# laboshinl/loam_velodyne

Measured on AMD Instinct MI355X. Metric: sweeps/sec (64-ring, 1M-pt map): feature extraction + odometry + scan-to-map registration, higher is better.
Workload: dtype f32

## Files before the change

loam_velodyne_amd/csrc/features.hip:

```cpp
#include "features.hpp"
#include "pinned_copy.hpp"
#include "scan.hpp"

namespace loamx {

__device__ inline float sqdiff3(const float4& a, const float4& b) {
  const float dx = a.x - b.x, dy = a.y - b.y, dz = a.z - b.z;
  return dx * dx + dy * dy + dz * dz;
}
__device__ inline float sqdiff3w(const float4& a, const float4& b, float wb) {
  const float dx = a.x - b.x * wb, dy = a.y - b.y * wb, dz = a.z - b.z * wb;
  return dx * dx + dy * dy + dz * dz;
}

struct RingLds {
  uint8_t* flags;
  float* c;
  uint32_t* sorted;
  int8_t* label;
};

__device__ inline void wave_lds_sync() { __builtin_amdgcn_fence(__ATOMIC_ACQ_REL, "workgroup"); }

__device__ inline void mark_as_picked(uint32_t scan_i, int cr, uint8_t* flags, const uint8_t* gaps, int lane) {
// ... 271 lines not shown
        if (!(ep > sp) || ep - sp + 1 < (unsigned long long)cr) simple = 0;
      }
      s_simple = simple && !force_sequential;
    }
    float* c = (float*)(wave_base + wid * wave_bytes);
    uint32_t* sorted = (uint32_t*)(c + nmax);
    int8_t* label = (int8_t*)(sorted + nmax);
    for (int jb = 0; jb < nreg; jb += FEAT_WAVES) {
      const int j = jb + wid;
      uint32_t n = 0, gsp = 0, scan_sp = 0;
      if (j < nreg) {
        const unsigned long long sp = ((s0 + cr) * (unsigned long long)(nreg - j) + (e0 - cr) * (unsigned long long)j) / nreg;
        const unsigned long long ep = ((s0 + cr) * (unsigned long long)(nreg - 1 - j) + (e0 - cr) * (unsigned long long)(j + 1)) / nreg - 1;
        if (ep > sp) {
          n = (uint32_t)(ep - sp + 1);
          gsp = base + (uint32_t)sp;
          scan_sp = (uint32_t)(sp - s0);
        }
      }
      if (lane == 0) { reg_n[wid] = n; reg_gsp[wid] = gsp; reg_scan[wid] = scan_sp; }
      for (uint32_t e = lane; e < n; e += 64) {
        c[e] = curv_all[scan_sp + e];
        label[e] = 0;
      }
      if (lane < 4 && n) c[n + lane] = __builtin_inff();
      __syncthreads();
      FT_TS(1);
      if (sortP == 64) wave_sort_curvature<1>(c, n, sorted, lane);
      else if (sortP == 128) wave_sort_curvature<2>(c, n, sorted, lane);
      else if (sortP == 256) wave_sort_curvature<4>(c, n, sorted, lane);
      else if (sortP == 512) wave_sort_curvature<8>(c, n, sorted, lane);
      else if (wid < (int)nwaves) {
        unsigned long long* keys = (unsigned long long*)(wave_base + nwaves * wave_bytes + (size_t)wid * sortP * 8);
        for (uint32_t e = lane; e < sortP; e += 64)
          keys[e] = e < n ? ((unsigned long long)__float_as_uint(c[e]) << 32) | e : ~0ull;
        wave_lds_sync();
        for (uint32_t k = 2; k <= sortP; k <<= 1) {
          for (uint32_t j = k >> 1; j > 0; j >>= 1) {
            for (uint32_t t = lane; t < sortP / 2; t += 64) {
              const uint32_t i = ((t / j) * 2 * j) + (t % j), l = i + j;
              const unsigned long long a = keys[i], b = keys[l];
              const bool up = (i & k) == 0;
              if ((a > b) == up) { keys[i] = b; keys[l] = a; }
            }
            wave_lds_sync();
          }
        }
        for (uint32_t e = lane; e < n; e += 64) sorted[e] = (uint32_t)keys[e];
      }
      __syncthreads();
      FT_TS(2);
      if (s_simple) {
        const uint32_t rn = reg_n[wid];
        if (rn) {
          if (wid == 0 && jb > 0)
            for (uint32_t e = lane; e < (uint32_t)cr && e < rn; e += 64) flags[reg_scan[0] + e] |= fwd[reg_scan[0] + e];
          wave_lds_sync();
          region_picks(P, cr, rn, reg_gsp[wid], reg_scan[wid], c, sorted, label, flags, fwd, gaps, pickS + (size_t)j * P.max_sharp,
                       pickLS + (size_t)j * P.max_less_sharp, pickF + (size_t)j * P.max_flat, rcnt[j], lane);
        }
        __syncthreads();
        if (wid == 0) {
          for (int w = 1; w < FEAT_WAVES && jb + w < nreg; w++) {
            const uint32_t rn2 = reg_n[w], rscan2 = reg_scan[w], rgsp2 = reg_gsp[w];
            const float* rc = (const float*)(wave_base + w * wave_bytes);
            const uint32_t* rsorted = (const uint32_t*)(rc + nmax);
            int8_t* rlabel = (int8_t*)(rsorted + nmax);
            const bool hit = lane < cr && (uint32_t)lane < rn2 && fwd[rscan2 + lane] != 0 && rlabel[lane] != 0;
            if (__ballot(hit)) {
              for (uint32_t e = lane; e < rn2; e += 64) {
                flags[rscan2 + e] = flags0[rscan2 + e] | (e < (uint32_t)cr ? fwd[rscan2 + e] : (uint8_t)0);
                rlabel[e] = 0;
              }
              for (uint32_t e = lane; e < (uint32_t)cr; e += 64) fwd[rscan2 + rn2 + e] = 0;
              wave_lds_sync();
              region_picks(P, cr, rn2, rgsp2, rscan2, rc, rsorted, rlabel, flags, fwd, gaps, pickS + (size_t)(jb + w) * P.max_sharp,
                           pickLS + (size_t)(jb + w) * P.max_less_sharp, pickF + (size_t)(jb + w) * P.max_flat, rcnt[jb + w], lane);
            }
          }
        }
      } else if (wid == 0) {
        for (int w = 0; w < FEAT_WAVES && jb + w < nreg; w++) {
          const uint32_t rn2 = reg_n[w];
          if (rn2 == 0) continue;
          const float* rc = (const float*)(wave_base + w * wave_bytes);
          const uint32_t* rsorted = (const uint32_t*)(rc + nmax);
          int8_t* rlabel = (int8_t*)(rsorted + nmax);
          region_picks(P, cr, rn2, reg_gsp[w], reg_scan[w], rc, rsorted, rlabel, flags, nullptr, gaps, pickS + (size_t)(jb + w) * P.max_sharp,
                       pickLS + (size_t)(jb + w) * P.max_less_sharp, pickF + (size_t)(jb + w) * P.max_flat, rcnt[jb + w], lane);
        }
      }
      __syncthreads();
      FT_TS(3);
      for (uint32_t e = lane; e < n; e += 64) lf_valid[gsp + e] = label[e] <= 0 ? 1 : 0;
      __syncthreads();
    }
  }
  if (wid == 0 && len > 2u * cr + 1u) {
    uint32_t* lists[3] = {pickS, pickLS, pickF};
    const uint32_t per[3] = {(uint32_t)P.max_sharp, (uint32_t)P.max_less_sharp, (uint32_t)P.max_flat};
    uint32_t tot[3] = {0, 0, 0};
    for (int j = 0; j < nreg; j++) {
#pragma unroll
      for (int q = 0; q < 3; q++) {
        const uint32_t cnt = rcnt[j][q], src = (uint32_t)j * per[q];
        if (src != tot[q]) {
          for (uint32_t k0 = 0; k0 < cnt; k0 += 64) {
            const uint32_t k = k0 + lane;
            const uint32_t v = k < cnt ? lists[q][src + k] : 0u;
            wave_lds_sync();
            if (k < cnt) lists[q][tot[q] + k] = v;
            wave_lds_sync();
          }
        }
        tot[q] += cnt;
      }
    }
    nS = tot[0]; nLS = tot[1]; nF = tot[2];
  }
  if (tid == 0) {
    cntS[r] = nS;
    cntLS[r] = nLS;
    cntF[r] = nF;
    npick[0] = nS; npick[1] = nLS; npick[2] = nF;
  }
  __syncthreads();
  for (uint32_t k = tid; k < npick[0]; k += blockDim.x) slotS[(size_t)r * capS + k] = cloud[pickS[k]];
  for (uint32_t k = tid; k < npick[1]; k += blockDim.x) slotLS[(size_t)r * capLS + k] = cloud[pickLS[k]];
  for (uint32_t k = tid; k < npick[2]; k += blockDim.x) slotF[(size_t)r * capF + k] = cloud[pickF[k]];
  FT_TS(4);
}

struct FeatRingLds {
  uint32_t flag_bytes, nmax, sortP, nwaves;
  size_t bytes;
};
constexpr size_t FEAT_LDS_STATIC = 1024;
constexpr size_t FEAT_LDS_MAX = 160 * 1024 - FEAT_LDS_STATIC;
static_assert(sizeof(uint32_t) * (3 * FEAT_WAVES + 3 + 64 * 3) + sizeof(int) <= FEAT_LDS_STATIC, "k_feat_ring's static LDS");

static FeatRingLds feat_ring_lds(uint32_t max_len, const FeatParams& p) {
  FeatRingLds r;
  const size_t caps = (size_t)(p.max_sharp + p.max_less_sharp + p.max_flat) * p.n_regions;
  r.flag_bytes = (max_len + 15u) & ~15u;
  r.nmax = (max_len / (uint32_t)p.n_regions + 8u + 15u) & ~15u;
  r.sortP = 64;
  while (r.sortP < r.nmax) r.sortP <<= 1;
  r.nwaves = (uint32_t)std::min(p.n_regions, FEAT_WAVES);
  r.bytes = ((8 * (size_t)r.flag_bytes + 4 * caps + 15) & ~(size_t)15) + (size_t)r.nwaves * r.nmax * (4 + 4 + 1) +
            (r.sortP > 512 ? (size_t)r.nwaves * r.sortP * 8 : 0) + 16;
  return r;
}

constexpr int LFV_THREADS = 1024;
constexpr uint32_t LFV_MAX = 4096;

__global__ __launch_bounds__(LFV_THREADS) void k_feat_lf_voxel(const float4* __restrict__ cloud, const uint32_t* __restrict__ ring_off,
                                                               const uint8_t* __restrict__ lf_valid, float inv_leaf, uint32_t P,
                                                               float4* __restrict__ slots, uint32_t* __restrict__ cnt) {
  extern __shared__ __attribute__((aligned(16))) char smem[];
  unsigned long long* keys = (unsigned long long*)smem;
  __shared__ uint32_t sc[17];
  __shared__ int mm[6];
  __shared__ uint32_t s_wcnt[LFV_THREADS / 64][256];
  __shared__ uint32_t s_base[256];
  const uint32_t r = blockIdx.x, tid = threadIdx.x;
  const uint32_t s0 = ring_off[r], len = ring_off[r + 1] - s0;
  if (tid < 3) mm[tid] = 2147483647;
  else if (tid < 6) mm[tid] = -2147483647 - 1;
  for (uint32_t k = tid; k < P; k += LFV_THREADS) keys[k] = ~0ull;
  __syncthreads();
  uint32_t base = 0;
  for (uint32_t b = 0; b < len; b += LFV_THREADS) {
    const uint32_t i = b + tid;
    const uint32_t v = (i < len && lf_valid[s0 + i]) ? 1u : 0u;
    uint32_t total;
    const uint32_t ex = block_excl_scan(v, sc, total);
    if (v) keys[base + ex] = i;
    base += total;
  }
  const uint32_t m = base;
  __syncthreads();
  {
    int lo[3] = {2147483647, 2147483647, 2147483647}, hi[3] = {-2147483647 - 1, -2147483647 - 1, -2147483647 - 1};
    for (uint32_t j = tid; j < m; j += LFV_THREADS) {
      const float4 p = cloud[s0 + (uint32_t)keys[j]];
      const int c[3] = {(int)floorf(p.x * inv_leaf), (int)floorf(p.y * inv_leaf), (int)floorf(p.z * inv_leaf)};
#pragma unroll
      for (int a = 0; a < 3; a++) { lo[a] = min(lo[a], c[a]); hi[a] = max(hi[a], c[a]); }
    }
#pragma unroll
    for (int off = 32; off > 0; off >>= 1) {
#pragma unroll
      for (int a = 0; a < 3; a++) {
        lo[a] = min(lo[a], __shfl_xor(lo[a], off, 64));
        hi[a] = max(hi[a], __shfl_xor(hi[a], off, 64));
      }
    }
    if ((tid & 63u) == 0) {
#pragma unroll
      for (int a = 0; a < 3; a++) { atomicMin(&mm[a], lo[a]); atomicMax(&mm[3 + a], hi[a]); }
    }
  }
  __syncthreads();
  const long long dx = (long long)mm[3] - mm[0] + 1, dy = (long long)mm[4] - mm[1] + 1, dz = (long long)mm[5] - mm[2] + 1;
  const bool pass = m > 0 && (dx > 2147483647LL || dy > 2147483647LL || dx * dy > 2147483647LL || dz > 2147483647LL / (dx * dy) + 1 || dx * dy * dz > 2147483647LL);
  for (uint32_t j = tid; j < m; j += LFV_THREADS) {
    const uint32_t li = (uint32_t)keys[j];
    unsigned long long k;
    if (pass) {
      k = (unsigned long long)j;
    } else {
      const float4 p = cloud[s0 + li];
      const int jx = (int)floorf(p.x * inv_leaf), jy = (int)floorf(p.y * inv_leaf), jz = (int)floorf(p.z * inv_leaf);
      k = (unsigned long long)((long long)(jx - mm[0]) + (long long)(jy - mm[1]) * dx + (long long)(jz - mm[2]) * dx * dy);
    }
    keys[j] = (k << 12) | li;
  }
  __syncthreads();
  unsigned long long* kb[2] = {keys, (unsigned long long*)(smem + (size_t)P * 8)};
  uint32_t npass = 0;
  if (!pass && m > 1) {
    const unsigned long long top = (unsigned long long)(dx * dy * dz - 1);
    const uint32_t bits = top ? 64u - (uint32_t)__builtin_clzll(top) : 0u;
    npass = (bits + 7u) / 8u;
  }
  {
    const uint32_t lane = tid & 63u, wid = tid >> 6;
    const uint32_t per_wave = ((m + LFV_THREADS - 1) / LFV_THREADS) * 64u;
    for (uint32_t ps = 0; ps < npass; ps++) {
      const uint32_t shift = 12u + 8u * ps;
      const unsigned long long* src = kb[ps & 1];
      unsigned long long* dst = kb[(ps & 1) ^ 1];
      for (uint32_t e = tid; e < (LFV_THREADS / 64) * 256; e += LFV_THREADS) (&s_wcnt[0][0])[e] = 0u;
      __syncthreads();
      unsigned long long key[4];
      uint32_t rank[4];
#pragma unroll
      for (int j = 0; j < 4; j++) {
        const uint32_t i = wid * per_wave + (uint32_t)j * 64u + lane;
        const bool in = (uint32_t)j * 64u < per_wave && i < m;
        key[j] = in ? src[i] : ~0ull;
        const uint32_t d = (uint32_t)((key[j] >> shift) & 255ull);
        unsigned long long mt = __ballot(in);
#pragma unroll
        for (int b = 0; b < 8; b++) {
          const unsigned long long bal = __ballot((d >> b) & 1u);
          mt &= ((d >> b) & 1u) ? bal : ~bal;
        }
        const unsigned long long below = mt & ((1ull << lane) - 1ull);
        const int leader = __builtin_ctzll(mt | (1ull << 63));
        uint32_t old = 0u;
        if (in && (int)lane == leader) {
          old = s_wcnt[wid][d];
          s_wcnt[wid][d] = old + (uint32_t)__popcll(mt);
        }
        old = __shfl(old, leader, 64);
        rank[j] = old + (uint32_t)__popcll(below);
        __builtin_amdgcn_wave_barrier();
      }
      __syncthreads();
      uint32_t run = 0;
      if (tid < 256) {
#pragma unroll
        for (int w = 0; w < LFV_THREADS / 64; w++) { const uint32_t c = s_wcnt[w][tid]; s_wcnt[w][tid] = run; run += c; }
      }
      uint32_t tot;
      const uint32_t ex = block_excl_scan(run, sc, tot);
      if (tid < 256) s_base[tid] = ex;
      __syncthreads();
#pragma unroll
      for (int j = 0; j < 4; j++) {
        const uint32_t i = wid * per_wave + (uint32_t)j * 64u + lane;
        if ((uint32_t)j * 64u < per_wave && i < m) {
          const uint32_t d = (uint32_t)((key[j] >> shift) & 255ull);
          dst[s_base[d] + s_wcnt[wid][d] + rank[j]] = key[j];
        }
      }
      __syncthreads();
    }
    if (npass & 1u) {
      for (uint32_t j = tid; j < m; j += LFV_THREADS) keys[j] = kb[1][j];
      __syncthreads();
    }
  }
  float4* sp = (float4*)(smem + (size_t)P * 8);
  for (uint32_t j = tid; j < m; j += LFV_THREADS) sp[j] = cloud[s0 + (uint32_t)(keys[j] & 4095ull)];
  __syncthreads();
  uint32_t obase = 0;
  for (uint32_t b = 0; b < m; b += LFV_THREADS) {
    const uint32_t j = b + tid;
    const bool head = j < m && (j == 0 || (keys[j] >> 12) != (keys[j - 1] >> 12));
    uint32_t total;
    const uint32_t ex = block_excl_scan(head ? 1u : 0u, sc, total);
    if (head) {
      const unsigned long long vk = keys[j] >> 12;
      float sx = 0.f, sy = 0.f, sz = 0.f, si = 0.f;
      uint32_t e = j;
      do {
        const float4 p = sp[e];
        sx += p.x; sy += p.y; sz += p.z; si += p.w;
        e++;
      } while (e < m && (keys[e] >> 12) == vk);
      const float c = (float)(e - j);
      slots[s0 + obase + ex] = make_float4(sx / c, sy / c, sz / c, si / c);
    }
    obase += total;
  }
  if (tid == 0) cnt[r] = obase;
}

__device__ inline uint32_t rings_before(const uint32_t* __restrict__ c, uint32_t r, int lane) {
  uint32_t part = 0u;
  for (uint32_t i = (uint32_t)lane; i < r; i += 64u) part += c[i];
#pragma unroll
  for (int d = 32; d > 0; d >>= 1) part += (uint32_t)__shfl_xor((int)part, d, 64);
  return part;
}
__global__ __launch_bounds__(64) void k_feat_compact(const float4* __restrict__ s0, const float4* __restrict__ s1, const float4* __restrict__ s2,
                                                     const uint32_t* __restrict__ c0, const uint32_t* __restrict__ c1, const uint32_t* __restrict__ c2,
                                                     uint32_t cap0, uint32_t cap1, uint32_t cap2, float4* __restrict__ o0, float4* __restrict__ o1,
                                                     float4* __restrict__ o2, uint32_t* __restrict__ offs, const uint32_t* __restrict__ sweep_ring_base,
                                                     uint32_t nsw, uint32_t* __restrict__ host_offs) {
  const uint32_t r = blockIdx.x, kind = blockIdx.y, nring = gridDim.x;
  const int lane = (int)threadIdx.x;
  const float4* s = kind == 0 ? s0 : (kind == 1 ? s1 : s2);
  const uint32_t* c = kind == 0 ? c0 : (kind == 1 ? c1 : c2);
  const uint32_t cap = kind == 0 ? cap0 : (kind == 1 ? cap1 : cap2);
  float4* o = kind == 0 ? o0 : (kind == 1 ? o1 : o2);
  const uint32_t dst = rings_before(c, r, lane), n = c[r];
  for (uint32_t k = (uint32_t)lane; k < n; k += 64u) o[dst + k] = s[(size_t)r * cap + k];
  if (lane == 0) {
    uint32_t* off = offs + (size_t)kind * (nsw + 1);
    uint32_t* hoff = host_offs ? host_offs + (size_t)kind * (nsw + 1) : nullptr;
    uint32_t lo = 0, hi = nsw + 1;
    while (lo < hi) { const uint32_t mid = (lo + hi) >> 1; if (sweep_ring_base[mid] < r) lo = mid + 1; else hi = mid; }
    for (uint32_t sw = lo; sw <= nsw && sweep_ring_base[sw] == r; sw++) { off[sw] = dst; if (hoff) hoff[sw] = dst; }
    if (r + 1 == nring)
      for (uint32_t sw = nsw; sweep_ring_base[sw] >= nring; sw--) { off[sw] = dst + n; if (hoff) hoff[sw] = dst + n; if (sw == 0) break; }
  }
}
__global__ __launch_bounds__(256) void k_feat_lf_compact(const float4* __restrict__ slots, const uint32_t* __restrict__ ring_off,
                                                         const uint32_t* __restrict__ cnt, uint32_t* __restrict__ lf_off, float4* __restrict__ out,
                                                         uint32_t* __restrict__ host_lf_off) {
  __shared__ uint32_t s_dst;
  const uint32_t r = blockIdx.x;
  if (threadIdx.x < 64) {
    const uint32_t d = rings_before(cnt, r, (int)threadIdx.x);
    if (threadIdx.x == 0) {
      s_dst = d;
      lf_off[r] = d;
      if (r + 1 == gridDim.x) lf_off[gridDim.x] = d + cnt[r];
      if (host_lf_off) {
        host_lf_off[r] = d;
        if (r + 1 == gridDim.x) host_lf_off[gridDim.x] = d + cnt[r];
      }
    }
  }
  __syncthreads();
  const uint32_t n = cnt[r], src = ring_off[r], dst = s_dst;
  for (uint32_t k = threadIdx.x; k < n; k += blockDim.x) out[dst + k] = slots[src + k];
}

FeatureExtractor::FeatureExtractor(int device, hipStream_t shared_stream) : device_(device) {
  select_device(device);
  if (shared_stream) {
    st_ = shared_stream;
  } else {
    LX_HIP(hipStreamCreateWithFlags(&st_, hipStreamNonBlocking));
    own_stream_ = true;
  }
  vox_.init(st_);
  h_bad_.reserve(16);
  h_bad_.p[0] = 0u;
  h_bad_.p[1] = 0u;
}

void FeatureExtractor::check_finite_input() {
  if (*(volatile uint32_t*)h_bad_.p) {
    *h_bad_.p = 0u;
    throw Error(LOAMX_E_INVALID, "a sweep holds non-finite coordinates (binned rings must be finite: BasicLaserOdometry.cpp:230 / MultiScanRegistration.cpp:187-196 drop such points before this stage)");
  }
}

FeatureExtractor::~FeatureExtractor() {
  if (ev_front_) (void)hipEventDestroy(ev_front_);
  if (ev_lf_) (void)hipEventDestroy(ev_lf_);
  if (own_stream_ && st_) (void)hipStreamDestroy(st_);
}

void FeatureExtractor::check_params_() const {
  LX_REQUIRE(params.curv_region >= 1 && params.curv_region <= 16, "curvature_region must be in [1,16]");
  LX_REQUIRE(params.n_regions >= 1 && params.n_regions <= 64, "n_feature_regions must be in [1,64]");
  LX_REQUIRE(params.max_sharp >= 0 && params.max_flat >= 0 && params.max_less_sharp >= params.max_sharp, "invalid pick limits");
  LX_REQUIRE(params.less_flat_leaf > 0.f, "less_flat_filter_size must be positive");
}

void FeatureExtractor::upload_async(uint32_t nsw, const loamx_cloud* clouds, const uint32_t* const* ring_size, const uint32_t* n_rings,
                                    hipStream_t copy_stream, hipEvent_t done, const std::function<bool(void*, const void*, size_t)>& big_copy) {
  LX_REQUIRE(nsw >= 1 && clouds && ring_size && n_rings && copy_stream && done, "invalid sweep batch");
  check_params_();
  LX_HIP(hipSetDevice(device_));
  bool packed = true;
  for (uint32_t s = 0; s < nsw; s++) {
    check_cloud(&clouds[s], false);
    uint32_t sum = 0;
    for (uint32_t r = 0; r < n_rings[s]; r++) sum += ring_size[s][r];
    LX_REQUIRE(sum == clouds[s].count, "ring sizes do not add up to the cloud size");
    packed = packed && clouds[s].stride == 16 && clouds[s].intensity_offset == 12;
  }
  layout_(nsw, ring_size, n_rings);
  allocate_(copy_stream);
  if (packed) {
    for (uint32_t s = 0; s < nsw;) {
      uint32_t e = s + 1;
      size_t cnt = clouds[s].count;
      while (e < nsw && (const char*)clouds[e].data == (const char*)clouds[s].data + sizeof(float4) * cnt) cnt += clouds[e++].count;
      if (cnt && !(big_copy && big_copy(cloud_.p + h_pt_base_[s], clouds[s].data, sizeof(float4) * cnt)))
        LX_HIP(hipMemcpyAsync(cloud_.p + h_pt_base_[s], clouds[s].data, sizeof(float4) * cnt, hipMemcpyHostToDevice, copy_stream));
      s = e;
    }
  } else {
    h_cloud_.reserve(n_ + 1);
    for (uint32_t s = 0; s < nsw; s++) pack_cloud(&clouds[s], h_cloud_.p + h_pt_base_[s]);
    if (n_) LX_HIP(hipMemcpyAsync(cloud_.p, h_cloud_.p, sizeof(float4) * n_, hipMemcpyHostToDevice, copy_stream));
  }
  LX_HIP(hipEventRecord(done, copy_stream));
}
void FeatureExtractor::upload_device(uint32_t nsw, const float4* d_src, const uint32_t* src_off, const uint32_t* const* ring_size,
                                     const uint32_t* n_rings, hipStream_t copy_stream, hipEvent_t done) {
  LX_REQUIRE(nsw >= 1 && d_src && src_off && ring_size && n_rings && copy_stream && done, "invalid sweep batch");
  check_params_();
  LX_HIP(hipSetDevice(device_));
  layout_(nsw, ring_size, n_rings);
  allocate_(copy_stream);
  for (uint32_t s = 0; s < nsw; s++) {
    const uint32_t cnt = h_pt_base_[s + 1] - h_pt_base_[s];
    if (cnt) LX_HIP(hipMemcpyAsync(cloud_.p + h_pt_base_[s], d_src + src_off[s], sizeof(float4) * cnt, hipMemcpyDeviceToDevice, copy_stream));
  }
  LX_HIP(hipEventRecord(done, copy_stream));
}
void FeatureExtractor::layout_(uint32_t nsw, const uint32_t* const* ring_size, const uint32_t* n_rings) {
  uint32_t longest = 0;
  for (uint32_t s = 0; s < nsw; s++)
    for (uint32_t r = 0; r < n_rings[s]; r++) longest = std::max(longest, ring_size[s][r]);
  LX_REQUIRE(feat_ring_lds(longest, params).bytes <= FEAT_LDS_MAX, "scan ring too long for the LDS staging of k_feat_ring (include/loamx.h)");
  nsw_ = nsw;
  h_ring_off_.assign(1, 0);
  h_ring_base_.assign(nsw + 1, 0);
  h_pt_base_.assign(nsw + 1, 0);
  h_ring_sweep_base_.clear();
  max_ring_len_ = 0;
  uint32_t pt = 0;
  for (uint32_t s = 0; s < nsw; s++) {
    uint32_t sum = 0;
    for (uint32_t r = 0; r < n_rings[s]; r++) {
      sum += ring_size[s][r];
      h_ring_off_.push_back(pt + sum);
      h_ring_sweep_base_.push_back(pt);
      max_ring_len_ = std::max(max_ring_len_, ring_size[s][r]);
    }
    pt += sum;
// ... 120 lines not shown
    imu_.fill_table(h_imu_d_.p, h_imu_f_.p, I);
    imu_dt_.reserve(2 * (size_t)H);
    imu_state_.reserve(9 * (size_t)H);
    imu_last_.reserve(1);
    h_imu_last_.reserve(1);
    LX_HIP(hipMemcpyAsync(imu_dt_.p, h_imu_d_.p, sizeof(double) * 2 * H, hipMemcpyHostToDevice, st_));
    LX_HIP(hipMemcpyAsync(imu_state_.p, h_imu_f_.p, sizeof(float) * 9 * H, hipMemcpyHostToDevice, st_));
    LX_HIP(hipMemsetAsync(imu_last_.p, 0, sizeof(ImuLast), st_));
    I.dt = imu_dt_.p;
    I.dstamp = imu_dt_.p + H;
    I.state = imu_state_.p;
  }
  return H;
}

void FeatureExtractor::finish_raw_(uint32_t n_scan_rings, uint32_t H) {
  LX_HIP(hipMemcpyAsync(h_raw_ring_cnt_.p, raw_ring_cnt_.p, sizeof(uint32_t) * n_scan_rings, hipMemcpyDeviceToHost, st_));
  if (H) LX_HIP(hipMemcpyAsync(h_imu_last_.p, imu_last_.p, sizeof(ImuLast), hipMemcpyDeviceToHost, st_));
  LX_HIP(hipStreamSynchronize(st_));
  if (H && h_imu_last_.p->valid) imu_.apply_last(*h_imu_last_.p);
  begin_sweep();
  const uint32_t* rs[1] = {h_raw_ring_cnt_.p};
  layout_(1, rs, &n_scan_rings);
  allocate_();
  LX_HIP(hipStreamSynchronize(st_));
}

void ImuTracker::update(double stamp, float roll, float pitch, float yaw, const float acc_in[3]) {
  State st;
  st.stamp = stamp; st.roll = HAngle(roll); st.pitch = HAngle(pitch); st.yaw = HAngle(yaw);
  st.acceleration = {acc_in[0], acc_in[1], acc_in[2]};
  if (!hist_.empty()) {
    HVec3 acc = st.acceleration;
    h_rot_zxy(acc, st.roll, st.pitch, st.yaw);
    const State& prev = hist_.back();
    const float dt = (float)(stamp - prev.stamp);
    st.position = {prev.position.x + prev.velocity.x * dt + 0.5f * acc.x * dt * dt, prev.position.y + prev.velocity.y * dt + 0.5f * acc.y * dt * dt,
                   prev.position.z + prev.velocity.z * dt + 0.5f * acc.z * dt * dt};
    st.velocity = {prev.velocity.x + acc.x * dt, prev.velocity.y + acc.y * dt, prev.velocity.z + acc.z * dt};
  }
  if (hist_.size() >= (size_t)std::max(history_size, 1)) hist_.pop_front();
  hist_.push_back(st);
}

void ImuTracker::interpolate_for_(float rel, State& out) {
  double td = (scan_time_ - hist_[idx_].stamp) + rel;
  while (idx_ < hist_.size() - 1 && td > 0) {
    idx_++;
    td = (scan_time_ - hist_[idx_].stamp) + rel;
  }
  if (idx_ == 0 || td > 0) {
    out = hist_[idx_];
  } else {
    const State &a = hist_[idx_], &b = hist_[idx_ - 1];
    const float ratio = (float)(-td / (a.stamp - b.stamp)), inv = 1 - ratio;
    out.roll = HAngle(a.roll.r * inv + b.roll.r * ratio);
    out.pitch = HAngle(a.pitch.r * inv + b.pitch.r * ratio);
    if (a.yaw.r - b.yaw.r > M_PI) out.yaw = HAngle((float)(a.yaw.r * inv + (b.yaw.r + 2 * M_PI) * ratio));
    else if (a.yaw.r - b.yaw.r < -M_PI) out.yaw = HAngle((float)(a.yaw.r * inv + (b.yaw.r - 2 * M_PI) * ratio));
    else out.yaw = HAngle(a.yaw.r * inv + b.yaw.r * ratio);
    out.velocity = {a.velocity.x * inv + b.velocity.x * ratio, a.velocity.y * inv + b.velocity.y * ratio, a.velocity.z * inv + b.velocity.z * ratio};
    out.position = {a.position.x * inv + b.position.x * ratio, a.position.y * inv + b.position.y * ratio, a.position.z * inv + b.position.z * ratio};
  }
}

void ImuTracker::begin_sweep() {
  scan_time_ = next_scan_time_;
  idx_ = 0;
  if (!hist_.empty()) interpolate_for_(0.f, start_);
  sweep_start_ = scan_time_;
  imu_trans_[0] = start_.pitch.r; imu_trans_[1] = start_.yaw.r; imu_trans_[2] = start_.roll.r;
  imu_trans_[3] = cur_.pitch.r; imu_trans_[4] = cur_.yaw.r; imu_trans_[5] = cur_.roll.r;
  HVec3 sh = shift_;
  h_rot_yxz(sh, -start_.yaw, -start_.pitch, -start_.roll);
  imu_trans_[6] = sh.x; imu_trans_[7] = sh.y; imu_trans_[8] = sh.z;
  HVec3 v{cur_.velocity.x - start_.velocity.x, cur_.velocity.y - start_.velocity.y, cur_.velocity.z - start_.velocity.z};
  h_rot_yxz(v, -start_.yaw, -start_.pitch, -start_.roll);
  imu_trans_[9] = v.x; imu_trans_[10] = v.y; imu_trans_[11] = v.z;
}

void ImuTracker::fill_table(double* h_d, float* h_f, ImuTable& I) const {
  const uint32_t H = (uint32_t)hist_.size();
  for (uint32_t j = 0; j < H; j++) {
    const State& s = hist_[j];
    h_d[j] = scan_time_ - s.stamp;
    h_d[H + j] = j ? s.stamp - hist_[j - 1].stamp : 1.0;
    float* o = h_f + 9 * (size_t)j;
    o[0] = s.roll.r; o[1] = s.pitch.r; o[2] = s.yaw.r;
    o[3] = s.position.x; o[4] = s.position.y; o[5] = s.position.z;
    o[6] = s.velocity.x; o[7] = s.velocity.y; o[8] = s.velocity.z;
  }
  I.H = H;
  I.idx0 = H ? (uint32_t)std::min(idx_, (size_t)H - 1) : 0u;
  const HAngle* sa[3] = {&start_.roll, &start_.pitch, &start_.yaw};
  for (int k = 0; k < 3; k++) { I.start_c[k] = sa[k]->c; I.start_s[k] = sa[k]->s; }
  I.start_pos[0] = start_.position.x; I.start_pos[1] = start_.position.y; I.start_pos[2] = start_.position.z;
  I.start_vel[0] = start_.velocity.x; I.start_vel[1] = start_.velocity.y; I.start_vel[2] = start_.velocity.z;
  I.rel_sweep_base = scan_time_ - sweep_start_;
}

void ImuTracker::apply_last(const ImuLast& L) {
  cur_.roll = HAngle(L.roll); cur_.pitch = HAngle(L.pitch); cur_.yaw = HAngle(L.yaw);
  cur_.position = {L.pos[0], L.pos[1], L.pos[2]};
  cur_.velocity = {L.vel[0], L.vel[1], L.vel[2]};
  shift_ = {L.shift[0], L.shift[1], L.shift[2]};
  idx_ = L.idx;
}

int FeatureExtractor::download_cloud(uint32_t sweep, loamx_cloud* full, uint32_t* ring_size_out) {
  LX_REQUIRE(sweep < nsw_, "sweep index out of range");
  const uint32_t r0 = h_ring_base_[sweep], r1 = h_ring_base_[sweep + 1];
  if (ring_size_out)
    for (uint32_t r = r0; r < r1; r++) ring_size_out[r - r0] = h_ring_off_[r + 1] - h_ring_off_[r];
  if (!full) return LOAMX_OK;
  check_cloud(full, false);
  const uint32_t a = h_pt_base_[sweep], b = h_pt_base_[sweep + 1];
  h_pack_.reserve((size_t)(b - a) + 2);
  if (b > a) LX_HIP(hipMemcpyAsync(h_pack_.p, cloud_.p + a, sizeof(float4) * (b - a), hipMemcpyDeviceToHost, st_));
  LX_HIP(hipStreamSynchronize(st_));
  return unpack_cloud(h_pack_.p, b - a, full);
}

void FeatureExtractor::run_async(bool mirror_offsets) {
  TraceRange trace_range("loamx:features:extract");
  LX_REQUIRE(nsw_ > 0, "run() before upload()");
  LX_HIP(hipSetDevice(device_));
  split_ = mirror_offsets && max_ring_len_ <= LFV_MAX;
  uint32_t* hmir = nullptr;
  if (split_) {
    h_mirror_off_.reserve(n_offsets());
    hmir = h_mirror_off_.p;
    if (!ev_front_) { LX_HIP(hipEventCreateWithFlags(&ev_front_, hipEventDisableTiming)); LX_HIP(hipEventCreateWithFlags(&ev_lf_, hipEventDisableTiming)); }
  }
  const int cr = params.curv_region;
  (void)cr;
  const uint32_t caps[3] = {(uint32_t)(params.max_sharp * params.n_regions), (uint32_t)(params.max_less_sharp * params.n_regions),
                            (uint32_t)(params.max_flat * params.n_regions)};
  const FeatRingLds L = feat_ring_lds(max_ring_len_, params);
  const size_t lds = L.bytes;
  LX_REQUIRE(lds <= FEAT_LDS_MAX, "internal: scan ring too long for the LDS staging of k_feat_ring");
  static const bool force_seq = diag_env("LOAMX_FEAT_SEQUENTIAL") && atoi(diag_env("LOAMX_FEAT_SEQUENTIAL")) != 0;
  if (lds > 64 * 1024)
    LX_HIP(hipFuncSetAttribute((const void*)k_feat_ring, hipFuncAttributeMaxDynamicSharedMemorySize, (int)lds));
  hipLaunchKernelGGL(k_feat_ring, dim3(nring_), dim3(64 * FEAT_WAVES), lds, st_, cloud_.p, ring_off_.p, ring_sweep_base_.p, params, L.flag_bytes, L.nmax,
                     L.sortP, L.nwaves, slots_[0].p, slots_[1].p, slots_[2].p, slot_cnt_[0].p, slot_cnt_[1].p, slot_cnt_[2].p, lf_valid_.p, force_seq ? 1 : 0,
                     h_bad_.p);
  hipLaunchKernelGGL(k_feat_compact, dim3(nring_, 3), dim3(64), 0, st_, slots_[0].p, slots_[1].p, slots_[2].p, slot_cnt_[0].p, slot_cnt_[1].p,
                     slot_cnt_[2].p, caps[0], caps[1], caps[2], out_[0].p, out_[1].p, out_[2].p, offs_.p, sweep_ring_base_.p, nsw_, hmir);
  if (split_) LX_HIP(hipEventRecord(ev_front_, st_));
  const float inv = 1.0f / params.less_flat_leaf;
  if (max_ring_len_ <= LFV_MAX) {
    uint32_t P = 2;
    while (P < max_ring_len_) P <<= 1;
    if ((size_t)P * 24 > 64 * 1024)
      LX_HIP(hipFuncSetAttribute((const void*)k_feat_lf_voxel, hipFuncAttributeMaxDynamicSharedMemorySize, (int)((size_t)P * 24)));
    hipLaunchKernelGGL(k_feat_lf_voxel, dim3(nring_), dim3(LFV_THREADS), (size_t)P * 24, st_, cloud_.p, ring_off_.p, lf_valid_.p, inv, P,
                       lf_slots_.p, lf_cnt_.p);
    hipLaunchKernelGGL(k_feat_lf_compact, dim3(nring_), dim3(256), 0, st_, lf_slots_.p, ring_off_.p, lf_cnt_.p, lf_off_(), lf_out_.p,
                       hmir ? hmir + (size_t)3 * off_stride_ : nullptr);
    if (split_) LX_HIP(hipEventRecord(ev_lf_, st_));
  } else {
    vox_.compute_ijk(cloud_.p, lf_valid_.p, n_, ring_off_.p, nring_, inv, inv);
    vox_.sort_reduce(cloud_.p, lf_valid_.p, n_, ring_off_.p, nring_, lf_out_.p, lf_off_());
  }
#ifdef LOAMX_PROF_FEAT
  {
    unsigned long long ts[8];
    LX_HIP(hipStreamSynchronize(st_));
    LX_HIP(hipMemcpyFromSymbol(ts, HIP_SYMBOL(g_feat_ts), sizeof(ts)));
    fprintf(stderr, "[feat_ring ts, 10ns ticks] load %lld  rank-sort %lld  picks %lld  tail %lld\n", (long long)(ts[1] - ts[0]), (long long)(ts[2] - ts[1]),
            (long long)(ts[3] - ts[2]), (long long)(ts[4] - ts[3]));
  }
#endif
  LX_HIP(hipGetLastError());
}

void FeatureExtractor::sync() {
  LX_HIP(hipStreamSynchronize(st_));
  vox_.check();
  check_finite_input();
}

__global__ __launch_bounds__(256) void k_feat_pack_host(const float4* __restrict__ o0, const float4* __restrict__ o1, const float4* __restrict__ o2,
                                                        const float4* __restrict__ lf, const uint32_t* __restrict__ off0,
                                                        const uint32_t* __restrict__ off1, const uint32_t* __restrict__ off2,
                                                        const uint32_t* __restrict__ lf_off, uint32_t sweep, uint32_t ring_a, uint32_t ring_b,
                                                        uint32_t capacity, float4* __restrict__ dst) {
  const uint32_t a0 = off0[sweep], n0 = off0[sweep + 1] - a0, a1 = off1[sweep], n1 = off1[sweep + 1] - a1;
  const uint32_t a2 = off2[sweep], n2 = off2[sweep + 1] - a2, a3 = lf_off[ring_a], n3 = lf_off[ring_b] - a3;
  const uint32_t total = n0 + n1 + n2 + n3;
  if (blockIdx.x == 0 && threadIdx.x == 0) {
    uint4 h = make_uint4(n0, n1, n2, n3);
    if (total > capacity) h = make_uint4(0xffffffffu, 0xffffffffu, 0xffffffffu, 0xffffffffu);
    *reinterpret_cast<uint4*>(dst) = h;
  }
  if (total > capacity) return;
  for (uint32_t i = blockIdx.x * blockDim.x + threadIdx.x; i < total; i += gridDim.x * blockDim.x) {
    float4 v;
    if (i < n0) v = o0[a0 + i];
    else if (i < n0 + n1) v = o1[a1 + (i - n0)];
    else if (i < n0 + n1 + n2) v = o2[a2 + (i - n0 - n1)];
    else v = lf[a3 + (i - n0 - n1 - n2)];
    dst[1 + i] = v;
  }
}

void FeatureExtractor::device_results(uint32_t sweep, const float4* ptr[4], uint32_t count[4]) {
  LX_REQUIRE(sweep < nsw_, "sweep index out of range");
  h_link_off_.reserve(n_offsets());
  LX_HIP(hipMemcpyAsync(h_link_off_.p, offs_.p, sizeof(uint32_t) * n_offsets(), hipMemcpyDeviceToHost, st_));
  LX_HIP(hipStreamSynchronize(st_));
  vox_.check();
  check_finite_input();
  const uint32_t* o = h_link_off_.p;
  for (int k = 0; k < 3; k++) {
    const uint32_t a = o[(size_t)k * off_stride_ + sweep], b = o[(size_t)k * off_stride_ + sweep + 1];
    ptr[k] = out_[k].p + a;
    count[k] = b - a;
  }
  const uint32_t* lf = o + (size_t)3 * off_stride_;
  const uint32_t a = lf[h_ring_base_[sweep]], b = lf[h_ring_base_[sweep + 1]];
  ptr[3] = lf_out_.p + a;
  count[3] = b - a;
}

void FeatureExtractor::device_results_front(uint32_t sweep, const float4* ptr[3], uint32_t count[3]) {
  LX_REQUIRE(sweep < nsw_, "sweep index out of range");
  LX_REQUIRE(split_, "internal: device_results_front() without run_async(true)");
  spin_event(ev_front_);
  check_finite_input();
  const uint32_t* o = h_mirror_off_.p;
  for (int k = 0; k < 3; k++) {
    const uint32_t a = o[(size_t)k * off_stride_ + sweep], b = o[(size_t)k * off_stride_ + sweep + 1];
    ptr[k] = out_[k].p + a;
    count[k] = b - a;
  }
}
void FeatureExtractor::device_results_lf(uint32_t sweep, const float4*& ptr, uint32_t& count) {
  LX_REQUIRE(sweep < nsw_, "sweep index out of range");
  LX_REQUIRE(split_, "internal: device_results_lf() without run_async(true)");
  spin_event(ev_lf_);
  const uint32_t* lf = h_mirror_off_.p + (size_t)3 * off_stride_;
  const uint32_t a = lf[h_ring_base_[sweep]], b = lf[h_ring_base_[sweep + 1]];
  ptr = lf_out_.p + a;
  count = b - a;
}

int FeatureExtractor::download(uint32_t sweep, loamx_cloud* sharp, loamx_cloud* less_sharp, loamx_cloud* flat, loamx_cloud* less_flat) {
  LX_REQUIRE(sweep < nsw_, "sweep index out of range");
  loamx_cloud* outs[4] = {sharp, less_sharp, flat, less_flat};
  for (auto* o : outs) if (o) check_cloud(o, false);
  const uint32_t n_pts = h_pt_base_[sweep + 1] - h_pt_base_[sweep];
  const uint32_t capacity = 4 * n_pts;
  h_pack_.reserve((size_t)capacity + 2);
  hipLaunchKernelGGL(k_feat_pack_host, dim3(std::min<uint32_t>((capacity + 1023) / 1024 + 1, 128u)), dim3(256), 0, st_, out_[0].p, out_[1].p, out_[2].p,
                     lf_out_.p, d_feat_off(0), d_feat_off(1), d_feat_off(2), lf_off_(), sweep, h_ring_base_[sweep], h_ring_base_[sweep + 1], capacity,
                     h_pack_.p);
  LX_HIP(hipStreamSynchronize(st_));
  vox_.check();
  check_finite_input();
  const uint32_t* hdr = reinterpret_cast<const uint32_t*>(h_pack_.p);
  LX_REQUIRE(hdr[0] != 0xffffffffu, "internal: the feature clouds of a sweep exceed four times its points");
  int rc = LOAMX_OK;
  const float4* src = h_pack_.p + 1;
  for (int k = 0; k < 4; k++) {
    if (outs[k]) {
      const int r = unpack_cloud(src, hdr[k], outs[k]);
      if (r != LOAMX_OK) rc = r;
    }
    src += hdr[k];
  }
  return rc;
}

}
```

Baseline: 16840.

## Restructure per-ring less-flat voxel kernel with LDS point staging and fewer block scans

Rewrites the per-ring voxel-downsample kernel to use 256 threads, each owning a contiguous chunk of points. Valid points are compacted with a single block scan and staged into LDS once, so the key and mean phases no longer reload from global memory. Head detection and the output base offsets use one wave-level scan instead of a block scan per chunk. The radix rank step drops the leader shuffle, and the mean accumulation is unrolled by four. It also adds an early exit for empty rings and optional profiling timestamps, at the cost of more LDS per block (32 bytes per slot instead of 24) and fewer threads per ring.

Result: no change. 16830 (-0.0%).

```diff
diff --git a/loam_velodyne_amd/csrc/features.hip b/loam_velodyne_amd/csrc/features.hip
--- a/loam_velodyne_amd/csrc/features.hip
+++ b/loam_velodyne_amd/csrc/features.hip
@@ -447,42 +447,76 @@
   return r;
 }
 
-constexpr int LFV_THREADS = 1024;
+constexpr int LFV_THREADS = 256;
 constexpr uint32_t LFV_MAX = 4096;
+constexpr int LFV_WAVES = LFV_THREADS / 64;
+constexpr int LFV_SLOTS = (int)LFV_MAX / LFV_THREADS;
+constexpr int LFV_LOADS = 8;
+static_assert(LFV_THREADS >= 256 && LFV_THREADS <= 1024 && LFV_WAVES * LFV_SLOTS == 64, "the 256 digits and the 64 head counts are scanned by one thread each");
+
+#ifdef LOAMX_PROF_FEAT
+__device__ unsigned long long g_lfv_ts[8];
+#define LFV_TS(k) do { if (blockIdx.x == 100 && threadIdx.x == 0) g_lfv_ts[k] = wall_clock64(); } while (0)
+#else
+#define LFV_TS(k) do { } while (0)
+#endif
 
 __global__ __launch_bounds__(LFV_THREADS) void k_feat_lf_voxel(const float4* __restrict__ cloud, const uint32_t* __restrict__ ring_off,
                                                                const uint8_t* __restrict__ lf_valid, float inv_leaf, uint32_t P,
                                                                float4* __restrict__ slots, uint32_t* __restrict__ cnt) {
   extern __shared__ __attribute__((aligned(16))) char smem[];
-  unsigned long long* keys = (unsigned long long*)smem;
+  float4* pts = (float4*)smem;
+  unsigned long long* kb0 = (unsigned long long*)(smem + (size_t)P * 16);
+  unsigned long long* kb1 = kb0 + P;
+  uint32_t* idx = (uint32_t*)kb1;
   __shared__ uint32_t sc[17];
   __shared__ int mm[6];
-  __shared__ uint32_t s_wcnt[LFV_THREADS / 64][256];
-  __shared__ uint32_t s_base[256];
-  const uint32_t r = blockIdx.x, tid = threadIdx.x;
+  __shared__ uint32_t s_wcnt[LFV_WAVES][256];
+  __shared__ uint32_t s_heads[64];
+  const uint32_t r = blockIdx.x, tid = threadIdx.x, lane = tid & 63u, wid = tid >> 6;
   const uint32_t s0 = ring_off[r], len = ring_off[r + 1] - s0;
+  LFV_TS(0);
   if (tid < 3) mm[tid] = 2147483647;
   else if (tid < 6) mm[tid] = -2147483647 - 1;
-  for (uint32_t k = tid; k < P; k += LFV_THREADS) keys[k] = ~0ull;
-  __syncthreads();
-  uint32_t base = 0;
-  for (uint32_t b = 0; b < len; b += LFV_THREADS) {
-    const uint32_t i = b + tid;
-    const uint32_t v = (i < len && lf_valid[s0 + i]) ? 1u : 0u;
-    uint32_t total;
-    const uint32_t ex = block_excl_scan(v, sc, total);
-    if (v) keys[base + ex] = i;
-    base += total;
-  }
-  const uint32_t m = base;
+  if (tid < 64) s_heads[tid] = 0u;
+  const uint32_t C = (len + LFV_THREADS - 1) / LFV_THREADS, first = tid * C;
+  uint32_t own = 0u;
+#pragma unroll
+  for (int c = 0; c < LFV_SLOTS; c++) {
+    const uint32_t i = first + (uint32_t)c;
+    if ((uint32_t)c < C && i < len && lf_valid[s0 + i]) own |= 1u << c;
+  }
+  uint32_t m;
+  {
+    uint32_t at = block_excl_scan((uint32_t)__popc(own), sc, m);
+    while (own) {
+      idx[at++] = first + (uint32_t)__builtin_ctz(own);
+      own &= own - 1u;
+    }
+  }
+  if (m == 0u) {
+    if (tid == 0) cnt[r] = 0u;
+    return;
+  }
   __syncthreads();
   {
     int lo[3] = {2147483647, 2147483647, 2147483647}, hi[3] = {-2147483647 - 1, -2147483647 - 1, -2147483647 - 1};
-    for (uint32_t j = tid; j < m; j += LFV_THREADS) {
-      const float4 p = cloud[s0 + (uint32_t)keys[j]];
-      const int c[3] = {(int)floorf(p.x * inv_leaf), (int)floorf(p.y * inv_leaf), (int)floorf(p.z * inv_leaf)};
-#pragma unroll
-      for (int a = 0; a < 3; a++) { lo[a] = min(lo[a], c[a]); hi[a] = max(hi[a], c[a]); }
+    for (uint32_t b = 0; b < m; b += LFV_LOADS * LFV_THREADS) {
+      uint32_t li[LFV_LOADS];
+      float4 p[LFV_LOADS];
+#pragma unroll
+      for (int k = 0; k < LFV_LOADS; k++) li[k] = idx[min(b + (uint32_t)k * LFV_THREADS + tid, m - 1u)];
+#pragma unroll
+      for (int k = 0; k < LFV_LOADS; k++) p[k] = cloud[s0 + li[k]];
+#pragma unroll
+      for (int k = 0; k < LFV_LOADS; k++) {
+        if (b + (uint32_t)k * LFV_THREADS + tid < m) {
+          pts[li[k]] = p[k];
+          const int c[3] = {(int)floorf(p[k].x * inv_leaf), (int)floorf(p[k].y * inv_leaf), (int)floorf(p[k].z * inv_leaf)};
+#pragma unroll
+          for (int a = 0; a < 3; a++) { lo[a] = min(lo[a], c[a]); hi[a] = max(hi[a], c[a]); }
+        }
+      }
     }
 #pragma unroll
     for (int off = 32; off > 0; off >>= 1) {
@@ -492,51 +526,54 @@
         hi[a] = max(hi[a], __shfl_xor(hi[a], off, 64));
       }
     }
-    if ((tid & 63u) == 0) {
+    if (lane == 0) {
 #pragma unroll
       for (int a = 0; a < 3; a++) { atomicMin(&mm[a], lo[a]); atomicMax(&mm[3 + a], hi[a]); }
     }
   }
   __syncthreads();
+  LFV_TS(1);
   const long long dx = (long long)mm[3] - mm[0] + 1, dy = (long long)mm[4] - mm[1] + 1, dz = (long long)mm[5] - mm[2] + 1;
-  const bool pass = m > 0 && (dx > 2147483647LL || dy > 2147483647LL || dx * dy > 2147483647LL || dz > 2147483647LL / (dx * dy) + 1 || dx * dy * dz > 2147483647LL);
+  const bool pass = dx > 2147483647LL || dy > 2147483647LL || dx * dy > 2147483647LL || dz > 2147483647LL / (dx * dy) + 1 || dx * dy * dz > 2147483647LL;
   for (uint32_t j = tid; j < m; j += LFV_THREADS) {
-    const uint32_t li = (uint32_t)keys[j];
+    const uint32_t li = idx[j];
     unsigned long long k;
     if (pass) {
       k = (unsigned long long)j;
     } else {
-      const float4 p = cloud[s0 + li];
+      const float4 p = pts[li];
       const int jx = (int)floorf(p.x * inv_leaf), jy = (int)floorf(p.y * inv_leaf), jz = (int)floorf(p.z * inv_leaf);
       k = (unsigned long long)((long long)(jx - mm[0]) + (long long)(jy - mm[1]) * dx + (long long)(jz - mm[2]) * dx * dy);
     }
-    keys[j] = (k << 12) | li;
+    kb0[j] = (k << 12) | li;
   }
   __syncthreads();
-  unsigned long long* kb[2] = {keys, (unsigned long long*)(smem + (size_t)P * 8)};
+  LFV_TS(2);
+#ifdef LOAMX_PROF_FEAT
+  if (blockIdx.x == 100 && tid == 0) g_lfv_ts[3] = g_lfv_ts[4] = g_lfv_ts[5] = g_lfv_ts[6] = 0ull;
+#endif
   uint32_t npass = 0;
   if (!pass && m > 1) {
     const unsigned long long top = (unsigned long long)(dx * dy * dz - 1);
     const uint32_t bits = top ? 64u - (uint32_t)__builtin_clzll(top) : 0u;
     npass = (bits + 7u) / 8u;
   }
-  {
-    const uint32_t lane = tid & 63u, wid = tid >> 6;
-    const uint32_t per_wave = ((m + LFV_THREADS - 1) / LFV_THREADS) * 64u;
-    for (uint32_t ps = 0; ps < npass; ps++) {
-      const uint32_t shift = 12u + 8u * ps;
-      const unsigned long long* src = kb[ps & 1];
-      unsigned long long* dst = kb[(ps & 1) ^ 1];
-      for (uint32_t e = tid; e < (LFV_THREADS / 64) * 256; e += LFV_THREADS) (&s_wcnt[0][0])[e] = 0u;
-      __syncthreads();
-      unsigned long long key[4];
-      uint32_t rank[4];
-#pragma unroll
-      for (int j = 0; j < 4; j++) {
+  const uint32_t per_wave = ((m + LFV_THREADS - 1) / LFV_THREADS) * 64u;
+  for (uint32_t ps = 0; ps < npass; ps++) {
+    const uint32_t shift = 12u + 8u * ps;
+    const unsigned long long* src = (ps & 1u) ? kb1 : kb0;
+    unsigned long long* dst = (ps & 1u) ? kb0 : kb1;
+    for (uint32_t e = tid; e < LFV_WAVES * 256; e += LFV_THREADS) (&s_wcnt[0][0])[e] = 0u;
+    __syncthreads();
+    uint32_t rank[LFV_SLOTS];
+#pragma unroll
+    for (int j = 0; j < LFV_SLOTS; j++) {
+      rank[j] = 0u;
+      if ((uint32_t)j * 64u < per_wave) {
         const uint32_t i = wid * per_wave + (uint32_t)j * 64u + lane;
-        const bool in = (uint32_t)j * 64u < per_wave && i < m;
-        key[j] = in ? src[i] : ~0ull;
-        const uint32_t d = (uint32_t)((key[j] >> shift) & 255ull);
+        const bool in = i < m;
+        const unsigned long long key = in ? src[i] : ~0ull;
+        const uint32_t d = (uint32_t)((key >> shift) & 255ull);
         unsigned long long mt = __ballot(in);
 #pragma unroll
         for (int b = 0; b < 8; b++) {
@@ -544,65 +581,84 @@
           mt &= ((d >> b) & 1u) ? bal : ~bal;
         }
         const unsigned long long below = mt & ((1ull << lane) - 1ull);
-        const int leader = __builtin_ctzll(mt | (1ull << 63));
-        uint32_t old = 0u;
-        if (in && (int)lane == leader) {
-          old = s_wcnt[wid][d];
-          s_wcnt[wid][d] = old + (uint32_t)__popcll(mt);
-        }
-        old = __shfl(old, leader, 64);
+        const uint32_t old = in ? s_wcnt[wid][d] : 0u;
+        __builtin_amdgcn_wave_barrier();
+        if (in && below == 0ull) s_wcnt[wid][d] = old + (uint32_t)__popcll(mt);
         rank[j] = old + (uint32_t)__popcll(below);
         __builtin_amdgcn_wave_barrier();
       }
-      __syncthreads();
-      uint32_t run = 0;
-      if (tid < 256) {
-#pragma unroll
-        for (int w = 0; w < LFV_THREADS / 64; w++) { const uint32_t c = s_wcnt[w][tid]; s_wcnt[w][tid] = run; run += c; }
-      }
-      uint32_t tot;
-      const uint32_t ex = block_excl_scan(run, sc, tot);
-      if (tid < 256) s_base[tid] = ex;
-      __syncthreads();
-#pragma unroll
-      for (int j = 0; j < 4; j++) {
-        const uint32_t i = wid * per_wave + (uint32_t)j * 64u + lane;
-        if ((uint32_t)j * 64u < per_wave && i < m) {
-          const uint32_t d = (uint32_t)((key[j] >> shift) & 255ull);
-          dst[s_base[d] + s_wcnt[wid][d] + rank[j]] = key[j];
-        }
-      }
-      __syncthreads();
-    }
-    if (npass & 1u) {
-      for (uint32_t j = tid; j < m; j += LFV_THREADS) keys[j] = kb[1][j];
-      __syncthreads();
-    }
-  }
-  float4* sp = (float4*)(smem + (size_t)P * 8);
-  for (uint32_t j = tid; j < m; j += LFV_THREADS) sp[j] = cloud[s0 + (uint32_t)(keys[j] & 4095ull)];
+    }
+    __syncthreads();
+    uint32_t run = 0, before[LFV_WAVES];
+#pragma unroll
+    for (int w = 0; w < LFV_WAVES; w++) {
+      before[w] = run;
+      if (tid < 256) run += s_wcnt[w][tid];
+    }
+    uint32_t tot;
+    const uint32_t ex = block_excl_scan(run, sc, tot);
+    if (tid < 256) {
+#pragma unroll
+      for (int w = 0; w < LFV_WAVES; w++) s_wcnt[w][tid] = ex + before[w];
+    }
+    __syncthreads();
+#pragma unroll
+    for (int j = 0; j < LFV_SLOTS; j++) {
+      const uint32_t i = wid * per_wave + (uint32_t)j * 64u + lane;
+      if ((uint32_t)j * 64u < per_wave && i < m) {
+        const unsigned long long key = src[i];
+        const uint32_t d = (uint32_t)((key >> shift) & 255ull);
+        dst[s_wcnt[wid][d] + rank[j]] = key;
+      }
+    }
+    __syncthreads();
+    LFV_TS(3 + ps);
+  }
+  const unsigned long long* keys = (npass & 1u) ? kb1 : kb0;
+  const uint32_t steps = (m + LFV_THREADS - 1) / LFV_THREADS;
+  uint32_t hmask = 0u;
+  for (uint32_t k = 0; k < steps; k++) {
+    const uint32_t j = k * LFV_THREADS + tid;
+    const bool head = j < m && (j == 0 || (keys[j] >> 12) != (keys[j - 1] >> 12));
+    const unsigned long long bal = __ballot(head);
+    if (head) hmask |= 1u << k;
+    if (lane == 0) s_heads[k * LFV_WAVES + wid] = (uint32_t)__popcll(bal);
+  }
   __syncthreads();
-  uint32_t obase = 0;
-  for (uint32_t b = 0; b < m; b += LFV_THREADS) {
-    const uint32_t j = b + tid;
-    const bool head = j < m && (j == 0 || (keys[j] >> 12) != (keys[j - 1] >> 12));
-    uint32_t total;
-    const uint32_t ex = block_excl_scan(head ? 1u : 0u, sc, total);
+  const uint32_t hc = s_heads[lane], hin = wave_incl_scan(hc, (int)lane), hex = hin - hc;
+  const uint32_t nvox = (uint32_t)__shfl((int)hin, 63, 64);
+  for (uint32_t k = 0; k < steps; k++) {
+    const bool head = (hmask >> k) & 1u;
+    const unsigned long long bal = __ballot(head);
+    const uint32_t base = (uint32_t)__shfl((int)hex, (int)(k * LFV_WAVES + wid), 64);
     if (head) {
+      const uint32_t j = k * LFV_THREADS + tid;
       const unsigned long long vk = keys[j] >> 12;
       float sx = 0.f, sy = 0.f, sz = 0.f, si = 0.f;
-      uint32_t e = j;
+      uint32_t e = j, n = 0u;
+      bool more = true;
       do {
-        const float4 p = sp[e];
-        sx += p.x; sy += p.y; sz += p.z; si += p.w;
-        e++;
-      } while (e < m && (keys[e] >> 12) == vk);
-      const float c = (float)(e - j);
-      slots[s0 + obase + ex] = make_float4(sx / c, sy / c, sz / c, si / c);
-    }
-    obase += total;
-  }
-  if (tid == 0) cnt[r] = obase;
+        unsigned long long kq[4];
+        float4 pq[4];
+#pragma unroll
+        for (int q = 0; q < 4; q++) kq[q] = keys[min(e + (uint32_t)q, m - 1u)];
+#pragma unroll
+        for (int q = 0; q < 4; q++) pq[q] = pts[(uint32_t)(kq[q] & 4095ull)];
+#pragma unroll
+        for (int q = 0; q < 4; q++) {
+          more = more && e + (uint32_t)q < m && (kq[q] >> 12) == vk;
+          const float ax = sx + pq[q].x, ay = sy + pq[q].y, az = sz + pq[q].z, ai = si + pq[q].w;
+          sx = more ? ax : sx; sy = more ? ay : sy; sz = more ? az : sz; si = more ? ai : si;
+          n += more ? 1u : 0u;
+        }
+        e += 4u;
+      } while (more);
+      const float c = (float)n;
+      slots[s0 + base + (uint32_t)__popcll(bal & ((1ull << lane) - 1ull))] = make_float4(sx / c, sy / c, sz / c, si / c);
+    }
+  }
+  if (tid == 0) cnt[r] = nvox;
+  LFV_TS(7);
 }
 
 __device__ inline uint32_t rings_before(const uint32_t* __restrict__ c, uint32_t r, int lane) {
@@ -1029,9 +1085,9 @@
   if (max_ring_len_ <= LFV_MAX) {
     uint32_t P = 2;
     while (P < max_ring_len_) P <<= 1;
-    if ((size_t)P * 24 > 64 * 1024)
-      LX_HIP(hipFuncSetAttribute((const void*)k_feat_lf_voxel, hipFuncAttributeMaxDynamicSharedMemorySize, (int)((size_t)P * 24)));
-    hipLaunchKernelGGL(k_feat_lf_voxel, dim3(nring_), dim3(LFV_THREADS), (size_t)P * 24, st_, cloud_.p, ring_off_.p, lf_valid_.p, inv, P,
+    if ((size_t)P * 32 > 64 * 1024)
+      LX_HIP(hipFuncSetAttribute((const void*)k_feat_lf_voxel, hipFuncAttributeMaxDynamicSharedMemorySize, (int)((size_t)P * 32)));
+    hipLaunchKernelGGL(k_feat_lf_voxel, dim3(nring_), dim3(LFV_THREADS), (size_t)P * 32, st_, cloud_.p, ring_off_.p, lf_valid_.p, inv, P,
                        lf_slots_.p, lf_cnt_.p);
     hipLaunchKernelGGL(k_feat_lf_compact, dim3(nring_), dim3(256), 0, st_, lf_slots_.p, ring_off_.p, lf_cnt_.p, lf_off_(), lf_out_.p,
                        hmir ? hmir + (size_t)3 * off_stride_ : nullptr);
@@ -1047,6 +1103,16 @@
     LX_HIP(hipMemcpyFromSymbol(ts, HIP_SYMBOL(g_feat_ts), sizeof(ts)));
     fprintf(stderr, "[feat_ring ts, 10ns ticks] load %lld  rank-sort %lld  picks %lld  tail %lld\n", (long long)(ts[1] - ts[0]), (long long)(ts[2] - ts[1]),
             (long long)(ts[3] - ts[2]), (long long)(ts[4] - ts[3]));
+    if (max_ring_len_ <= LFV_MAX) {
+      LX_HIP(hipMemcpyFromSymbol(ts, HIP_SYMBOL(g_lfv_ts), sizeof(ts)));
+      fprintf(stderr, "[feat_lf_voxel ts, 10ns ticks] compact+load %lld  bounds+keys %lld  radix passes", (long long)(ts[1] - ts[0]), (long long)(ts[2] - ts[1]));
+      unsigned long long prev = ts[2];
+      for (int k = 3; k < 7; k++) {
+        if (ts[k] > prev) { fprintf(stderr, " %lld", (long long)(ts[k] - prev)); prev = ts[k]; }
+        else fprintf(stderr, " -");
+      }
+      fprintf(stderr, "  heads+means %lld\n", (long long)(ts[7] - prev));
+    }
   }
 #endif
   LX_HIP(hipGetLastError());
```
